# fxcawley/nanoSandbox

Hardware: AMD Instinct MI355X
Metric: tokens/sec (whole node) GPT-2 124M DDP (higher is better)
Workload: dtype bf16

## Files before the change

csrc/kernels/flash_attn.hip:

```cpp
#include "common.h"

#include <type_traits>

#ifndef NSA_FA_F16
#define NSA_FA_F16 0
#endif
#if NSA_FA_F16
#define NSA_FA_SYM(name) name##_h
#else
#define NSA_FA_SYM(name) name
#endif
constexpr bool kFaH = NSA_FA_F16 != 0;

namespace {

__device__ __forceinline__ __bf16 fa_elt(float v) { return f2frag<kFaH>(v); }
__device__ __forceinline__ float fa_f(__bf16 v) { return e2f<kFaH>(__builtin_bit_cast(uint16_t, v)); }

constexpr float kLog2e = 1.4426950408889634f;
#ifndef ATTN_ORDER_DEFAULT
#define ATTN_ORDER_DEFAULT 0
#endif

template <int D>
// ... 4 lines not shown
};

template <int BITS>
__device__ __forceinline__ int bitrev(int k) {
  if constexpr (BITS == 2) return ((k & 1) << 1) | ((k >> 1) & 1);
  else if constexpr (BITS == 3) return ((k & 1) << 2) | (k & 2) | ((k >> 2) & 1);
  else return (int)(__builtin_bitreverse32((uint32_t)k) >> 28);
}

template <int D>
__device__ __forceinline__ int swz(int row, int chunk) {
  using G = Geo<D>;
  const int key = bitrev<G::BITS>((row / G::RPB) & (G::CPR - 1));
  return row * (D * 2) + ((chunk ^ key) << 4);
}

__device__ __forceinline__ uint4 lds_b128(const char* base, int off) {
  return *reinterpret_cast<const uint4*>(base + off);
}

__device__ __forceinline__ s16x4 lds_tr(const char* base, int off) {
  return __builtin_amdgcn_ds_read_tr16_b64_v4i16((__attribute__((address_space(3))) s16x4*)(base + off));
}

__device__ __forceinline__ bf16x8 cat_tr(s16x4 a, s16x4 b) {
  typedef short s16x8 __attribute__((ext_vector_type(8)));
  s16x8 v = __builtin_shufflevector(a, b, 0, 1, 2, 3, 4, 5, 6, 7);
  return __builtin_bit_cast(bf16x8, v);
}

__device__ __forceinline__ bf16x8 as_frag(uint4 u) { return __builtin_bit_cast(bf16x8, u); }

__device__ __forceinline__ f32x16 mfma(bf16x8 a, bf16x8 b, f32x16 c) { return mfma32e<kFaH>(a, b, c); }

__device__ __forceinline__ void attn_order(int n_tiles, int BH, int order, int& bh, int& t) {
  const int v = blockIdx.x;
  if (order == 0) {
    t = v / BH;
    bh = v % BH;
    return;
  }
  if (order == 2) {
    bh = v / n_tiles;
    t = v % n_tiles;
    return;
  }
  const int total = n_tiles * BH;
  const int xcd = v % 8, q = total / 8, r = total % 8;
  const int u = (xcd < r ? xcd * (q + 1) : r * (q + 1) + (xcd - r) * q) + v / 8;
  bh = u / n_tiles;
  t = u % n_tiles;
}

enum { FWD_AUTO = 0, FWD_V1 = 1, FWD_V5 = 5 };
enum { BWD_V1 = 1, BWD_V2 = 2, BWD_V3 = 3 };
struct FlashConfig {
  int fwd, bwd, order;
};
}
NSA_API void* nsa_flash_config_ptr();
namespace {
#if NSA_FA_F16
FlashConfig& flash_config() { return *static_cast<FlashConfig*>(nsa_flash_config_ptr()); }
#else
FlashConfig& flash_config() {
  static FlashConfig c = [] {
    FlashConfig d{FWD_AUTO, BWD_V3, ATTN_ORDER_DEFAULT};
    if (const char* e = getenv("NSA_FLASH_FWD"))
      d.fwd = (e[0] == 'v' && (e[1] == '1' || e[1] == '5')) ? e[1] - '0' : FWD_AUTO;
    if (const char* e = getenv("NSA_FLASH_BWD"))
      d.bwd = (e[0] == 'v' && e[1] >= '1' && e[1] <= '3') ? e[1] - '0' : BWD_V3;
    if (const char* e = getenv("NSA_ATTN_ORDER")) d.order = (e[0] >= '0' && e[0] <= '2') ? e[0] - '0' : 0;
    return d;
  }();
  return c;
}
#endif
int attn_order_env() { return flash_config().order; }

__device__ __forceinline__ int acc_row(int i, int h) { return (i & 3) + 8 * (i >> 2) + 4 * h; }

__device__ __forceinline__ float fast_exp2(float x) { return __builtin_amdgcn_exp2f(x); }

template <int D>
__device__ __forceinline__ bf16x8 tr_frag(const char* tile, int r0, int r1, int col_base, int lane) {
  const int g = lane >> 4, ig = lane & 15;
  const int q = ig >> 2, p = ig & 3;
  const int col = col_base + 16 * (g & 1) + 4 * p;
  const int chunk = col >> 3, half = (col >> 2) & 1;
  const s16x4 a = lds_tr(tile, swz<D>(r0 + q, chunk) + half * 8);
  const s16x4 b = lds_tr(tile, swz<D>(r1 + q, chunk) + half * 8);
  return cat_tr(a, b);
}

template <int W>
__device__ __forceinline__ bf16x8 tr_frag_w(const char* tile, int r0, int r1, int col_base, int lane) {
  return tr_frag<W>(tile, r0, r1, col_base, lane);
}

#ifndef NSA_FA_M0KEEP
#define NSA_FA_M0KEEP 0
#endif
__device__ __forceinline__ void glds16s(uint32_t voff, const void* sbase, uint32_t lds_dst) {
  if constexpr (NSA_FA_M0KEEP) {
    unsigned keep;
    asm volatile("s_mov_b32 %0, m0\n\ts_mov_b32 m0, %3\n\ts_nop 0\n\tglobal_load_lds_dwordx4 %1, %2\n\ts_mov_b32 m0, %0"
                 : "=&s"(keep)
                 : "v"(voff), "s"(sbase), "s"(lds_dst)
                 : "memory");
  } else {
    asm volatile("s_mov_b32 m0, %2\n\ts_nop 0\n\tglobal_load_lds_dwordx4 %0, %1" ::"v"(voff), "s"(sbase), "s"(lds_dst)
                 : "memory");
  }
}
__device__ __forceinline__ void glds16(const void* gsrc, uint32_t lds_dst) {
  if constexpr (NSA_FA_M0KEEP) {
    unsigned keep;
    asm volatile("s_mov_b32 %0, m0\n\ts_mov_b32 m0, %2\n\ts_nop 0\n\tglobal_load_lds_dwordx4 %1, off\n\ts_mov_b32 m0, %0"
                 : "=&s"(keep)
                 : "v"(gsrc), "s"(lds_dst)
                 : "memory");
  } else {
// ... 521 lines not shown
  asm volatile("s_waitcnt vmcnt(0)" ::: "memory");
  __syncthreads();
  for (int j = 0; j < n_tiles; j += 2) {
    issue(min(j + 2, n_tiles - 1), (j + 2) % 4);
    issue(min(j + 3, n_tiles - 1), (j + 3) % 4);
#pragma unroll
    for (int u = 0; u < 2; ++u) {
      const int jj = j + u;
      if (NSA_PROBE_SKIP_TILE && jj == 1) continue;
      if (jj < n_tiles) {
        const int kv0 = jj * BN;
        const char* kt = smem + (jj % 4) * TILE_BYTES;
        const char* vt = smem + (4 + jj % 4) * TILE_BYTES;
        if (kv0 + BN - 1 <= q0w) {
          if (!(fast && fwd_tile5<false>(kt, vt, qf, o, l_i, kv0, qposA, h, r, lane, scale_log2))) {
            if (fast) fwd5_to_exact(o, m_i, l_i, sl_exact);
            fast = false;
            fwd_tile2<false, false>(kt, vt, qf, o, m_i, l_i, kv0, qposA, h, r, lane, sl_exact, dr);
          }
        } else if (kv0 <= q0w + 63) {
          if (!(fast && fwd_tile5<true>(kt, vt, qf, o, l_i, kv0, qposA, h, r, lane, scale_log2))) {
            if (fast) fwd5_to_exact(o, m_i, l_i, sl_exact);
            fast = false;
            fwd_tile2<true, false>(kt, vt, qf, o, m_i, l_i, kv0, qposA, h, r, lane, sl_exact, dr);
          }
        }
      }
    }
    asm volatile("s_waitcnt vmcnt(0)" ::: "memory");
    __syncthreads();
  }
#pragma unroll
  for (int blk = 0; blk < 2; ++blk) {
    const int qp = qposA + 32 * blk;
    if (qp < T) {
      const float inv_l = 1.0f / l_i[blk];
      bf16_t* orow = out + ((int64_t)b * T + qp) * C + hh * D;
#pragma unroll
      for (int dt = 0; dt < 2; ++dt) {
#pragma unroll
        for (int g = 0; g < 4; ++g) {
          const int d = 32 * dt + 8 * g + 4 * h;
          uint2 u;
          u.x = pk2<kFaH>(o[blk][dt][4 * g + 0] * inv_l, o[blk][dt][4 * g + 1] * inv_l);
          u.y = pk2<kFaH>(o[blk][dt][4 * g + 2] * inv_l, o[blk][dt][4 * g + 3] * inv_l);
          *reinterpret_cast<uint2*>(orow + d) = u;
        }
      }
      if (h == 0) lse_out[(int64_t)bh * T + qp] = (m_i[blk] * sl_exact + __log2f(l_i[blk])) * 0.6931471805599453f;
    }
  }
}

template <int D>
__global__ __launch_bounds__(256) void flash_bwd_pre_kernel(const bf16_t* __restrict__ o,
                                                           const bf16_t* __restrict__ dout,
                                                           float* __restrict__ delta, int B, int T, int H) {
  constexpr int LPR = D / 8;
  const int C = H * D;
  const int64_t gid = (int64_t)blockIdx.x * 256 + threadIdx.x;
  const int64_t row = gid / LPR;
  const int sub = gid % LPR;
  if (row >= (int64_t)B * T * H) return;
  const int hh = row % H;
  const int64_t bt = row / H;
  const int t = bt % T, b = bt / T;
  const int64_t off = bt * C + hh * D + sub * 8;
  float a[8], g[8];
  load8e<kFaH>(o + off, a);
  load8e<kFaH>(dout + off, g);
  float s = 0.0f;
#pragma unroll
  for (int j = 0; j < 8; ++j) s += a[j] * g[j];
#pragma unroll
  for (int k = LPR / 2; k > 0; k >>= 1) s += __shfl_xor(s, k, 64);
  if (sub == 0) delta[((int64_t)b * H + hh) * T + t] = s;
}

template <int D>
struct BwdGeo {
  static constexpr int KB = D == 64 ? 256 : 128;
  static constexpr int NW = KB / 32;
};

template <bool MASK, bool DROP>
__device__ __forceinline__ void bwd_probs(const f32x16& sacc, const f32x16& dpacc, const float* lse2_s,
                                          const float* delta_s, int qrow0, int qbase_pos, int kpos, int h,
                                          float scale_log2, const DropArgs& dr, bf16x8 (&pfr)[2],
                                          bf16x8 (&dsfr)[2]) {
#pragma unroll
  for (int g = 0; g < 4; ++g) {
    const float4 l4 = *reinterpret_cast<const float4*>(lse2_s + qrow0 + 8 * g + 4 * h);
    const float4 d4 = *reinterpret_cast<const float4*>(delta_s + qrow0 + 8 * g + 4 * h);
    const float lv[4] = {l4.x, l4.y, l4.z, l4.w};
    const float dlv[4] = {d4.x, d4.y, d4.z, d4.w};
#pragma unroll
    for (int e = 0; e < 4; ++e) {
      const int i = 4 * g + e;
      const int q = qbase_pos + 8 * g + 4 * h + e;
      float p = fast_exp2(sacc[i] * scale_log2 - lv[e]);
      if constexpr (MASK) {
        if (kpos > q || q >= dr.T) p = 0.0f;
      }
      float dp = dpacc[i];
      float pd = p;
      if constexpr (DROP) {
// ... 391 lines not shown
  for (int kb = 0; kb < NKB; ++kb) {
    sacc[kb] = row_consts(ld, h);
#pragma unroll
    for (int ks = 0; ks < 4; ++ks) sacc[kb] = mfma(qa[ks], kf[kb][ks], sacc[kb]);
  }
#pragma unroll
  for (int kb = 0; kb < NKB; ++kb) {
    pacc[kb] = DROP ? f32x16{} : row_consts(ld + 32, h);
#pragma unroll
    for (int ks = 0; ks < 4; ++ks) pacc[kb] = mfma(da[ks], vf[kb][ks], pacc[kb]);
  }
  bf16x8 pfr[NKB][2], dsfr[NKB][2];
#pragma unroll
  for (int kb = 0; kb < NKB; ++kb) {
    const int key = kw + 32 * kb + r;
    f32x16 nd;
    if constexpr (DROP) nd = row_consts(ld + 32, h);
    float pv[16], dsv[16];
#pragma unroll
    for (int i = 0; i < 16; ++i) {
      float p = fast_exp2(sacc[kb][i] * scale_log2);
      if constexpr (MASK) p = key > q0 + acc_row(i, h) ? 0.0f : p;
      if constexpr (DROP) {
        const int q = q0 + acc_row(i, h);
        const uint64_t id = ((uint64_t)dr.bh * dr.T + (uint64_t)q) * (uint64_t)dr.T + (uint64_t)key;
        const bool keep = nsa_keep(dr.seed, id, dr.thresh);
        pv[i] = keep ? p * dr.scale : 0.0f;
        dsv[i] = p * ((keep ? pacc[kb][i] * dr.scale : 0.0f) + nd[i]);
      } else {
        pv[i] = p;
        dsv[i] = p * pacc[kb][i];
      }
    }
    pack16(pv, pfr[kb]);
    pack16(dsv, dsfr[kb]);
  }
#pragma unroll
  for (int s = 0; s < 2; ++s) {
    const int r0 = 16 * s + 4 * h;
#pragma unroll
    for (int dt = 0; dt < 2; ++dt) {
      const bf16x8 doa = tr_frag<D>(dot, r0, r0 + 8, 32 * dt, lane);
#pragma unroll
      for (int kb = 0; kb < NKB; ++kb) dv[kb][dt] = mfma(doa, pfr[kb][s], dv[kb][dt]);
      const bf16x8 qta = tr_frag<D>(qt, r0, r0 + 8, 32 * dt, lane);
#pragma unroll
      for (int kb = 0; kb < NKB; ++kb) dk[kb][dt] = mfma(qta, dsfr[kb][s], dk[kb][dt]);
    }
  }
}

#ifndef NSA_DKDV_NS
#define NSA_DKDV_NS 4
#endif

template <int NKB, int NW, bool DROP, int G = 1>
__global__ __launch_bounds__(NW * 64, NKB == 2 ? 1 : (NW == 8 ? 1 : 2)) void flash_bwd_dkdv2_kernel(
    const bf16_t* __restrict__ qkv, const bf16_t* __restrict__ dout, const float* __restrict__ nls,
    const float* __restrict__ nd, bf16_t* __restrict__ dqkv, int B, int T, int H, float scale,
    float scale_log2, uint32_t drop_thresh, float drop_scale, uint64_t seed, int order) {
  constexpr int D = 64;
  constexpr int KPW = 32 * NKB;
  constexpr int KWG = KPW * NW;
  constexpr int SLOT = V2Geo<NW>::SLOT;
  constexpr int NS = G > 1 ? 2 * G : NSA_DKDV_NS, LA = NS - 1;
  __shared__ __attribute__((aligned(16))) char smem[NS * SLOT];
  const int C = H * D;
  const int64_t row_stride = 3 * (int64_t)C;
  const int BH = B * H;
  int bh, kbw;
  attn_order((T + KWG - 1) / KWG, BH, order, bh, kbw);
  const int b = bh / H, hh = bh % H;
  const int tid = threadIdx.x, lane = tid & 63;
  const int w = __builtin_amdgcn_readfirstlane(tid >> 6);
  const int h = lane >> 5, r = lane & 31;
  const int k0 = kbw * KWG;
  const int kw = k0 + KPW * w;
  const bf16_t* base = qkv + (int64_t)b * T * row_stride;
  const bf16_t* qbase = base + hh * D;
  const bf16_t* kbase = base + C + hh * D;
  const bf16_t* vbase = base + 2 * C + hh * D;
  const bf16_t* dobase = dout + (int64_t)b * T * C + hh * D;
  const float* nls_bh = nls + (int64_t)bh * T;
  const float* nd_bh = nd + (int64_t)bh * T;
  const DropArgs dr{drop_thresh, drop_scale, nsa_seed(seed), bh, T};
  const uint32_t lds0 =
      __builtin_amdgcn_readfirstlane((uint32_t)(uintptr_t)((__attribute__((address_space(3))) char*)smem));

  const int s_first = k0 / 32;
  const int n_mine = T / 32 - s_first;

  const int piece = NW == 4 ? w : (w & 3);
  const int prow = 8 * piece + (lane >> 3);
  const int pch = (lane & 7) ^ bitrev<3>((prow >> 1) & 7);
  const bf16_t* qsrc = qbase + (int64_t)prow * row_stride + pch * 8;
  const bf16_t* dosrc = dobase + (int64_t)prow * C + pch * 8;
  const float* csrc = (h == 0 ? nls_bh : nd_bh) + r;
  auto issue = [&](int s, int slot) {
    const uint32_t sb = lds0 + (uint32_t)(slot * SLOT);
    if (NW == 4 || w < 4) glds16(qsrc + (int64_t)s * 32 * row_stride, sb + (uint32_t)(8 * piece * 128));
    if (NW == 4 || w >= 4) glds16(dosrc + (int64_t)s * 32 * C, sb + (uint32_t)(V2_QT + 8 * piece * 128));
    glds4(csrc + s * 32, sb + (uint32_t)(2 * V2_QT + w * 256));
  };

  for (int j = 0; j < (G > 1 ? G : LA) && j < n_mine; ++j) issue(s_first + j, j);

  bf16x8 kf[NKB][4], vf[NKB][4];
#pragma unroll
  for (int kb = 0; kb < NKB; ++kb) {
    int kc = kw + 32 * kb + r;
    kc = kc < T ? kc : T - 1;
#pragma unroll
    for (int ks = 0; ks < 4; ++ks) {
      kf[kb][ks] = as_frag(*reinterpret_cast<const uint4*>(kbase + (int64_t)kc * row_stride + 16 * ks + 8 * h));
      vf[kb][ks] = as_frag(*reinterpret_cast<const uint4*>(vbase + (int64_t)kc * row_stride + 16 * ks + 8 * h));
    }
  }
#pragma unroll
  for (int kb = 0; kb < NKB; ++kb)
    asm volatile("" ::"v"(kf[kb][0]), "v"(kf[kb][1]), "v"(kf[kb][2]), "v"(kf[kb][3]), "v"(vf[kb][0]),
                 "v"(vf[kb][1]), "v"(vf[kb][2]), "v"(vf[kb][3]));
  f32x16 dk[NKB][2], dv[NKB][2];
#pragma unroll
  for (int kb = 0; kb < NKB; ++kb)
#pragma unroll
    for (int dt = 0; dt < 2; ++dt) {
      dk[kb][dt] = f32x16{};
      dv[kb][dt] = f32x16{};
    }

  auto open_slice = [&](int j) {
    vm_wait(V2Geo<NW>::PIECES * min(LA - 1, n_mine - 1 - j));
    asm volatile("s_waitcnt lgkmcnt(0)" ::: "memory");
    __builtin_amdgcn_s_barrier();
    if (j + LA < n_mine) issue(s_first + j + LA, (j + LA) % NS);
  };
  auto slice_full = [&](int j) {
    auto f = [&](auto slot) {
      const char* qt = smem + decltype(slot)::value * SLOT;
      dkdv_slice<NKB, false, DROP>(qt, qt + V2_QT, reinterpret_cast<const float*>(qt + 2 * V2_QT) + w * 64, kf,
                                   vf, dk, dv, (s_first + j) * 32, kw, h, r, lane, scale_log2, dr);
    };
    slot_dispatch<0, NS>(j % NS, f);
  };
  auto slice_diag = [&](int j) {
    auto f = [&](auto slot) {
      const char* qt = smem + decltype(slot)::value * SLOT;
      dkdv_slice<NKB, true, DROP>(qt, qt + V2_QT, reinterpret_cast<const float*>(qt + 2 * V2_QT) + w * 64, kf,
                                  vf, dk, dv, (s_first + j) * 32, kw, h, r, lane, scale_log2, dr);
    };
    slot_dispatch<0, NS>(j % NS, f);
  };

  const int j_diag = min(NKB * w, n_mine);
  const int j_full = min(NKB * w + NKB, n_mine);
  if constexpr (G > 1) {
    for (int j = 0; j < n_mine; j += G) {
      asm volatile("s_waitcnt vmcnt(0) lgkmcnt(0)" ::: "memory");
      __builtin_amdgcn_s_barrier();
#pragma unroll
      for (int u = 0; u < G; ++u)
        if (j + G + u < n_mine) issue(s_first + j + G + u, (j + G + u) % NS);
#pragma unroll
      for (int u = 0; u < G; ++u) {
        const int jj = j + u;
        if (jj >= j_full) {
          if (jj < n_mine) slice_full(jj);
        } else if (jj >= j_diag) {
          slice_diag(jj);
        }
      }
    }
  } else {
    int j = 0;
    for (; j < j_diag; ++j) open_slice(j);
    for (; j < j_full; ++j) {
      open_slice(j);
      slice_diag(j);
    }
    for (; j < n_mine; ++j) {
      open_slice(j);
      slice_full(j);
    }
  }

#pragma unroll
  for (int kb = 0; kb < NKB; ++kb) {
    const int kpos = kw + 32 * kb + r;
    if (kpos < T) {
      bf16_t* krow = dqkv + ((int64_t)b * T + kpos) * row_stride + C + hh * D;
      bf16_t* vrow = krow + C;
#pragma unroll
      for (int dt = 0; dt < 2; ++dt) {
#pragma unroll
        for (int g = 0; g < 4; ++g) {
          const int d = 32 * dt + 8 * g + 4 * h;
          uint2 uk, uv;
          uk.x = cvt2(dk[kb][dt][4 * g + 0] * scale, dk[kb][dt][4 * g + 1] * scale);
          uk.y = cvt2(dk[kb][dt][4 * g + 2] * scale, dk[kb][dt][4 * g + 3] * scale);
          uv.x = cvt2(dv[kb][dt][4 * g + 0], dv[kb][dt][4 * g + 1]);
          uv.y = cvt2(dv[kb][dt][4 * g + 2], dv[kb][dt][4 * g + 3]);
          *reinterpret_cast<uint2*>(krow + d) = uk;
          *reinterpret_cast<uint2*>(vrow + d) = uv;
        }
      }
    }
  }
}

constexpr int DQ2_T = 64 * 64 * 2;
#ifndef NSA_DQ2_NS
#define NSA_DQ2_NS 4
#endif
#ifndef NSA_DQ2_OCC
#define NSA_DQ2_OCC 2
#endif

template <bool MASK, bool DROP>
__device__ __forceinline__ void dq2_tile(const char* kt, const char* vt, const bf16x8 (&qf)[4],
                                         const bf16x8 (&gf)[4], const f32x16& ndt, f32x16 (&dq)[2], float lse2,
                                         int kv0, int qpos, int h, int r, int lane, float scale_log2,
                                         const DropArgs& dr) {
  constexpr int D = 64;
  f32x16 st[2], pt[2];
#pragma unroll
// ... 128 lines not shown
    auto f = [&](auto slot) {
      const char* kt = smem + decltype(slot)::value * SLOT;
      dq2_tile<false, DROP>(kt, kt + DQ2_T, qf, gf, ndt, dq, lse2, 64 * j, qpos, h, r, lane, scale_log2, dr);
    };
    slot_dispatch<0, NS>(j % NS, f);
  };
  auto tile_diag = [&](int j) {
    auto f = [&](auto slot) {
      const char* kt = smem + decltype(slot)::value * SLOT;
      dq2_tile<true, DROP>(kt, kt + DQ2_T, qf, gf, ndt, dq, lse2, 64 * j, qpos, h, r, lane, scale_log2, dr);
    };
    slot_dispatch<0, NS>(j % NS, f);
  };

  const int m = min(q0w / 64, n_tiles);
  int j = 0;
  for (; j < m; ++j) {
    open_tile(j);
    tile_full(j);
  }
  if (j < n_tiles) {
    open_tile(j);
    tile_diag(j);
    ++j;
  }
  for (; j < n_tiles; ++j) open_tile(j);

  if (qpos < T) {
    bf16_t* qrow = dqkv + ((int64_t)b * T + qpos) * row_stride + hh * D;
#pragma unroll
    for (int dt = 0; dt < 2; ++dt) {
#pragma unroll
      for (int g = 0; g < 4; ++g) {
        const int d = 32 * dt + 8 * g + 4 * h;
        uint2 u;
        u.x = cvt2(dq[dt][4 * g + 0] * scale, dq[dt][4 * g + 1] * scale);
        u.y = cvt2(dq[dt][4 * g + 2] * scale, dq[dt][4 * g + 3] * scale);
        *reinterpret_cast<uint2*>(qrow + d) = u;
      }
    }
  }
}

template <int D>
hipError_t fwd_launch(const void* qkv, void* out, void* lse, int B, int T, int H, float scale, float p,
                      uint64_t seed, hipStream_t s) {
  const int n_qt = (T + 127) / 128;
  const uint32_t th = p > 0.0f ? nsa_drop_thresh(p) : 0u;
  const float dscale = p > 0.0f ? 1.0f / (1.0f - p) : 1.0f;
  const int order = attn_order_env();
  if constexpr (D == 64) {
    const int n_qt5 = (T + 255) / 256;
    const int sel = flash_config().fwd;
    if (!th && (sel == FWD_V5 || (sel == FWD_AUTO && (int64_t)n_qt5 * B * H >= 4096))) {
      flash_fwd5_kernel<<<n_qt5 * B * H, 256, 0, s>>>((const bf16_t*)qkv, (bf16_t*)out, (float*)lse, B, T, H,
                                                      scale * kLog2e, order);
      return hipGetLastError();
    }
    if (th)
      flash_fwd_kernel<D, true, true><<<n_qt * B * H, 256, 0, s>>>((const bf16_t*)qkv, (bf16_t*)out, (float*)lse, B,
                                                                   T, H, scale * kLog2e, th, dscale, seed, order);
    else
      flash_fwd_kernel<D, false, true><<<n_qt * B * H, 256, 0, s>>>((const bf16_t*)qkv, (bf16_t*)out, (float*)lse,
                                                                    B, T, H, scale * kLog2e, th, dscale, seed, order);
    return hipGetLastError();
  }
  if (th)
    flash_fwd_kernel<D, true><<<n_qt * B * H, 256, 0, s>>>((const bf16_t*)qkv, (bf16_t*)out, (float*)lse, B, T, H,
                                                           scale * kLog2e, th, dscale, seed, order);
  else
    flash_fwd_kernel<D, false><<<n_qt * B * H, 256, 0, s>>>((const bf16_t*)qkv, (bf16_t*)out, (float*)lse, B, T, H,
                                                            scale * kLog2e, th, dscale, seed, order);
  return hipGetLastError();
}

template <int D>
hipError_t bwd_launch(const void* qkv, const void* o, const void* dout, const void* lse, void* delta, void* dqkv,
                      int B, int T, int H, float scale, float p, uint64_t seed, hipStream_t s) {
  const int64_t threads = (int64_t)B * T * H * (D / 8);
  flash_bwd_pre_kernel<D><<<(unsigned)((threads + 255) / 256), 256, 0, s>>>((const bf16_t*)o, (const bf16_t*)dout,
                                                                             (float*)delta, B, T, H);
  hipError_t e = hipGetLastError();
  if (e != hipSuccess) return e;
  const uint32_t th = p > 0.0f ? nsa_drop_thresh(p) : 0u;
  const float dscale = p > 0.0f ? 1.0f / (1.0f - p) : 1.0f;
  const int n_kb = (T + BwdGeo<D>::KB - 1) / BwdGeo<D>::KB;
  const dim3 grid(n_kb * B * H), block(BwdGeo<D>::NW * 64);
#define NSA_BWD_ARGS                                                                                        \
  (const bf16_t*)qkv, (const bf16_t*)dout, (const float*)lse, (const float*)delta, (bf16_t*)dqkv, B, T, H, \
      scale, scale * kLog2e, th, dscale, seed
  if (th) flash_bwd_kernel<D, true><<<grid, block, 0, s>>>(NSA_BWD_ARGS);
  else flash_bwd_kernel<D, false><<<grid, block, 0, s>>>(NSA_BWD_ARGS);
#undef NSA_BWD_ARGS
  e = hipGetLastError();
  if (e != hipSuccess) return e;
  const int n_qt = (T + 127) / 128;
  if (th)
    flash_bwd_dq_kernel<D, true><<<n_qt * B * H, 256, 0, s>>>(
        (const bf16_t*)qkv, (const bf16_t*)dout, (const float*)lse, (const float*)delta, (bf16_t*)dqkv, B, T, H,
        scale, scale * kLog2e, th, dscale, seed, 1.0f);
  else
    flash_bwd_dq_kernel<D, false><<<n_qt * B * H, 256, 0, s>>>(
        (const bf16_t*)qkv, (const bf16_t*)dout, (const float*)lse, (const float*)delta, (bf16_t*)dqkv, B, T, H,
        scale, scale * kLog2e, th, dscale, seed, 1.0f);
  return hipGetLastError();
}

// ... 17 lines not shown
  hipError_t e = hipGetLastError();
  if (e != hipSuccess) return e;
  const int n_kb = (T + 127) / 128;
  if (flash_config().bwd == BWD_V3 && !th)
    flash_bwd_dkdv2_kernel<1, 4, false, 2><<<n_kb * B * H, 256, 0, s>>>((const bf16_t*)qkv, (const bf16_t*)dout,
                                                                          nls, nd, (bf16_t*)dqkv, B, T, H, scale,
                                                                          scale * kLog2e, th, dscale, seed, order);
  else if (th)
    flash_bwd_dkdv2_kernel<1, 4, true><<<n_kb * B * H, 256, 0, s>>>((const bf16_t*)qkv, (const bf16_t*)dout, nls, nd,
                                                                   (bf16_t*)dqkv, B, T, H, scale, scale * kLog2e, th,
                                                                   dscale, seed, order);
  else
    flash_bwd_dkdv2_kernel<1, 4, false><<<n_kb * B * H, 256, 0, s>>>((const bf16_t*)qkv, (const bf16_t*)dout, nls,
                                                                    nd, (bf16_t*)dqkv, B, T, H, scale, scale * kLog2e,
                                                                    th, dscale, seed, order);
  return hipGetLastError();
}

}

NSA_API hipError_t NSA_FA_SYM(nsa_flash_bwd2)(const void* qkv, const void* o, const void* dout, const void* lse, void* ws,
                                  void* dqkv, int B, int T, int H, int D, float scale, float p, uint64_t seed,
                                  hipStream_t s) {
  if (D == 64 && T % 32 == 0 && flash_config().bwd >= BWD_V2)
    return bwd2_launch64(qkv, o, dout, lse, ws, dqkv, B, T, H, scale, p, seed, s);
  switch (D) {
    case 32: return bwd_launch<32>(qkv, o, dout, lse, ws, dqkv, B, T, H, scale, p, seed, s);
    case 64: return bwd_launch<64>(qkv, o, dout, lse, ws, dqkv, B, T, H, scale, p, seed, s);
    case 128: return bwd_launch<128>(qkv, o, dout, lse, ws, dqkv, B, T, H, scale, p, seed, s);
    default: return hipErrorInvalidValue;
  }
}

#define NSA_FA_RNG(NAME) NSA_DEFINE_RNG_ADVANCE(NAME)
NSA_FA_RNG(NSA_FA_SYM(nsa_rng_advance_attn))


NSA_API hipError_t NSA_FA_SYM(nsa_flash_fwd)(const void* qkv, void* out, void* lse, int B, int T, int H, int D, float scale,
                                 float p, uint64_t seed, hipStream_t s) {
  switch (D) {
    case 32: return fwd_launch<32>(qkv, out, lse, B, T, H, scale, p, seed, s);
    case 64: return fwd_launch<64>(qkv, out, lse, B, T, H, scale, p, seed, s);
    case 128: return fwd_launch<128>(qkv, out, lse, B, T, H, scale, p, seed, s);
    default: return hipErrorInvalidValue;
  }
}

#if !NSA_FA_F16
NSA_API void* nsa_flash_config_ptr() { return &flash_config(); }

NSA_API int nsa_flash_set_variant(int fwd, int bwd, int order) {
  FlashConfig& c = flash_config();
  const int prev = c.fwd | (c.bwd << 4) | (c.order << 8);
  if (fwd == FWD_AUTO || fwd == FWD_V1 || fwd == FWD_V5) c.fwd = fwd;
  if (bwd >= BWD_V1 && bwd <= BWD_V3) c.bwd = bwd;
  if (order >= 0 && order <= 2) c.order = order;
  return prev;
}
#endif
```

nanosandbox_amd/build.py:

```python

from __future__ import annotations

import argparse
import glob
import os
import shutil
import subprocess
import sys
from concurrent.futures import ThreadPoolExecutor

ROOT = os.path.dirname(os.path.dirname(os.path.abspath(__file__)))
CSRC = os.path.join(ROOT, "csrc")
LIB_DIR = os.path.join(ROOT, "nanosandbox_amd", "lib")
BUILD_DIR = os.path.join(ROOT, "build", "obj")
ARCH = os.environ.get("NSA_OFFLOAD_ARCH", "gfx950")

KERNEL_LIB = os.path.join(LIB_DIR, "libnsa_kernels.so")
RUNTIME_LIB = os.path.join(LIB_DIR, "libnsa_runtime.so")
BIN_DIR = os.path.join(ROOT, "nanosandbox_amd", "bin")
RCCL_BENCH = os.path.join(BIN_DIR, "rccl_bench")


def _hipcc():
    for c in (os.environ.get("HIPCC"), "/opt/rocm/bin/hipcc", shutil.which("hipcc")):
        if c and os.path.exists(c):
            return c
    raise FileNotFoundError("hipcc not found (ROCm 7.x expected under /opt/rocm)")


def _newer(target, sources):
    if not os.path.exists(target):
        return True
    t = os.path.getmtime(target)
    return any(os.path.getmtime(s) > t for s in sources)


def _run(cmd):
    r = subprocess.run(cmd, capture_output=True, text=True)
    if r.returncode != 0:
        raise RuntimeError(f"build failed: {' '.join(cmd)}\n{r.stdout}\n{r.stderr}")
    return r


FILE_FLAGS = {"flash_attn.hip": ["-fno-slp-vectorize"], "flash_attn_f16.hip": ["-fno-slp-vectorize"]}


def build_kernels(force=False, jobs=8, verbose=True, defines=(), lib_path=KERNEL_LIB, obj_dir=BUILD_DIR,
                  file_flags=None):
    srcs = sorted(glob.glob(os.path.join(CSRC, "kernels", "*.hip")))
    headers = glob.glob(os.path.join(CSRC, "kernels", "*.h"))
    if not force and not _newer(lib_path, srcs + headers + [os.path.abspath(__file__)]):
        return lib_path
    os.makedirs(obj_dir, exist_ok=True)
    os.makedirs(os.path.dirname(lib_path), exist_ok=True)
    hipcc = _hipcc()
    flags = [f"--offload-arch={ARCH}", "-O3", "-std=c++17", "-fPIC", "-fvisibility=hidden",
             "-munsafe-fp-atomics", "-I", os.path.join(CSRC, "kernels"), *[f"-D{d}" for d in defines]]

    def deps(src):
        out = []
        for line in open(src):
            if line.startswith('#include "') and line.rstrip().endswith('.hip"'):
                out.append(os.path.join(os.path.dirname(src), line.split('"')[1]))
        return out

    ff = FILE_FLAGS if file_flags is None else file_flags

    def compile_one(src):
        obj = os.path.join(obj_dir, os.path.basename(src) + ".o")
        if force or _newer(obj, [src] + headers + deps(src) + [os.path.abspath(__file__)]):
            _run([hipcc, *flags, *ff.get(os.path.basename(src), []), "-c", src, "-o", obj])
            if verbose:
                print(f"  [hipcc {ARCH}] {os.path.relpath(src, ROOT)}")
        return obj

    with ThreadPoolExecutor(max_workers=max(1, jobs)) as ex:
        objs = list(ex.map(compile_one, srcs))
    tmp = lib_path + ".tmp"
    _run([hipcc, f"--offload-arch={ARCH}", "-shared", "-fPIC", *objs, "-o", tmp])
    os.replace(tmp, lib_path)
    if verbose:
        print(f"built {os.path.relpath(lib_path, ROOT)}")
    return lib_path


def build_variant(name, defines, force=False, jobs=8, verbose=True, file_flags=None):
    vdir = os.path.join(ROOT, "build", "variants", name)
    return build_kernels(force=force, jobs=jobs, verbose=verbose, defines=defines,
                         lib_path=os.path.join(vdir, "libnsa_kernels.so"), obj_dir=os.path.join(vdir, "obj"),
                         file_flags=file_flags)


def build_runtime(force=False, verbose=True):
    srcs = sorted(glob.glob(os.path.join(CSRC, "runtime", "*.cpp")))
    if not srcs:
        return None
    if not force and not _newer(RUNTIME_LIB, srcs):
        return RUNTIME_LIB
    os.makedirs(LIB_DIR, exist_ok=True)
    cxx = os.environ.get("CXX", "g++")
    tmp = RUNTIME_LIB + ".tmp"
    _run([cxx, "-O3", "-std=c++17", "-fPIC", "-shared", "-pthread", *srcs, "-o", tmp])
    os.replace(tmp, RUNTIME_LIB)
    if verbose:
        print(f"built {os.path.relpath(RUNTIME_LIB, ROOT)}")
    return RUNTIME_LIB


def build_tools(force=False, verbose=True):
    src = os.path.join(CSRC, "comm", "rccl_bench.cpp")
    if not os.path.exists(src):
        return None
    if not force and not _newer(RCCL_BENCH, [src]):
        return RCCL_BENCH
    os.makedirs(BIN_DIR, exist_ok=True)
    rocm = os.environ.get("ROCM_PATH", "/opt/rocm")
    tmp = RCCL_BENCH + ".tmp"
    _run([_hipcc(), "-O2", "-std=c++17", "-I", os.path.join(rocm, "include"), src, "-L", os.path.join(rocm, "lib"),
          "-lrccl", f"-Wl,-rpath,{os.path.join(rocm, 'lib')}", "-o", tmp])
    os.replace(tmp, RCCL_BENCH)
    if verbose:
        print(f"built {os.path.relpath(RCCL_BENCH, ROOT)}")
    return RCCL_BENCH


def build_all(force=False, jobs=8, verbose=True):
    build_runtime(force=force, verbose=verbose)
    build_tools(force=force, verbose=verbose)
    return build_kernels(force=force, jobs=jobs, verbose=verbose)


def main(argv=None):
    ap = argparse.ArgumentParser()
    ap.add_argument("--force", action="store_true")
    ap.add_argument("--jobs", type=int, default=min(8, os.cpu_count() or 1))
    ap.add_argument("--variant", nargs="+", metavar=("NAME", "DEFINE"),
                    help="build an A/B probe variant: NAME followed by preprocessor defines")
    ap.add_argument("--no-file-flags", action="store_true",
                    help="with --variant: compile every source with the common flags only (no FILE_FLAGS)")
    a = ap.parse_args(argv)
    if a.variant:
        print(build_variant(a.variant[0], a.variant[1:], force=a.force, jobs=a.jobs,
                            file_flags={} if a.no_file_flags else None))
        return 0
    build_all(force=a.force, jobs=a.jobs)


if __name__ == "__main__":
    sys.exit(main())
```

nanosandbox_amd/ops/functional.py:

```python

from __future__ import annotations

import contextlib
import math
import os
from typing import NamedTuple

import torch
import torch.nn.functional as F

from . import _lib
from . import gemm as _gemm
from . import gemm_dispatch as _gd

BF16 = torch.bfloat16
F16 = torch.float16
F32 = torch.float32
KDT = (BF16, F16)


def _sym(name, dtype):
    return name + "_h" if dtype == F16 else name


# ... 557 lines not shown

def mlp(x, w_fc, b_fc, w_proj, b_proj, recompute=False):
    if x.is_cuda and x.dtype in KDT:
        return MLPFn.apply(x, w_fc, b_fc, w_proj, b_proj, recompute)
    return linear(gelu(linear(x, w_fc, b_fc)), w_proj, b_proj)



_INV_SQRT2 = 1.0 / math.sqrt(2.0)
_INV_SQRT2PI = 1.0 / math.sqrt(2.0 * math.pi)


class GeluFn(torch.autograd.Function):
    @staticmethod
    def forward(ctx, x):
        ctx.save_for_backward(x)
        if _kern(x):
            x = x.contiguous()
            y = torch.empty_like(x)
            _lib.call(_sym("nsa_gelu_fwd", x.dtype), _lib.ptr(x), _lib.ptr(y), x.numel(), _lib.stream())
            return y
        return F.gelu(x.float()).to(x.dtype)

    @staticmethod
    def backward(ctx, dy):
        (x,) = ctx.saved_tensors
        if _kern(dy):
            dy = dy.contiguous()
            dx = torch.empty_like(x)
            _lib.call(_sym("nsa_gelu_bwd", dy.dtype), _lib.ptr(dy), _lib.ptr(x), _lib.ptr(dx), x.numel(), _lib.stream())
            return dx
        xf = x.float()
        cdf = 0.5 * (1.0 + torch.erf(xf * _INV_SQRT2))
        pdf = torch.exp(-0.5 * xf * xf) * _INV_SQRT2PI
        return (dy.float() * (cdf + xf * pdf)).to(dy.dtype)


def gelu(x):
    return GeluFn.apply(x)



def _attn_reference(q, k, v, p, seed):
    T, D = q.shape[-2], q.shape[-1]
    att = (q @ k.transpose(-2, -1)) * (1.0 / math.sqrt(D))
    mask = torch.ones(T, T, dtype=torch.bool, device=q.device).tril()
    att = att.masked_fill(~mask, float("-inf"))
    att = torch.softmax(att, dim=-1)
    if p > 0:
        att = att * _cpu_keep_mask(att.shape, p, seed, att.device) / (1.0 - p)
    return att @ v


_FLASH_FWD = {"auto": 0, "v1": 1, "v5": 5}
_FLASH_BWD = {"v1": 1, "v2": 2, "v3": 3}


@contextlib.contextmanager
def flash_variant(fwd: str | None = None, bwd: str | None = None, order: int | None = None):
    prev = _lib.call_ret("nsa_flash_set_variant", _FLASH_FWD[fwd] if fwd else -1, _FLASH_BWD[bwd] if bwd else -1,
                         -1 if order is None else int(order))
    try:
        yield
    finally:
        _lib.call_ret("nsa_flash_set_variant", prev & 0xF, (prev >> 4) & 0xF, (prev >> 8) & 0xF)


class AttentionFn(torch.autograd.Function):
    @staticmethod
    def forward(ctx, qkv, n_head, p):
        B, T, C3 = qkv.shape
        C = C3 // 3
        H = n_head
        D = C // H
        seed = new_seed() if p > 0 else 0
        ctx.meta = (B, T, H, D, p, seed)
        scale = 1.0 / math.sqrt(D)
        ctx.kern = _kern(qkv)
        if ctx.kern:
            assert D in (32, 64, 128), "flash kernel supports head_dim 32/64/128"
            qkv = qkv.contiguous()
            y = torch.empty(B, T, C, device=qkv.device, dtype=qkv.dtype)
            lse = torch.empty(B, H, T, device=qkv.device, dtype=F32)
            _lib.call(_sym("nsa_flash_fwd", qkv.dtype), _lib.ptr(qkv), _lib.ptr(y), _lib.ptr(lse), B, T, H, D,
                      scale, p, seed, _lib.stream())
            ctx.save_for_backward(qkv, y, lse)
            return y
        q, k, v = qkv.float().view(B, T, 3, H, D).permute(2, 0, 3, 1, 4)
        y = _attn_reference(q, k, v, p, seed).transpose(1, 2).reshape(B, T, C)
        ctx.save_for_backward(qkv)
        return y.to(qkv.dtype)

    @staticmethod
    def backward(ctx, dy):
        B, T, H, D, p, seed = ctx.meta
        C = H * D
        if ctx.kern:
            qkv, y, lse = ctx.saved_tensors
            dy = dy.contiguous()
            dqkv = torch.empty_like(qkv)
            ws = torch.empty(2, B, H, T, device=dy.device, dtype=F32)
            dy = dy.to(qkv.dtype)
            _lib.call(_sym("nsa_flash_bwd2", qkv.dtype), _lib.ptr(qkv), _lib.ptr(y), _lib.ptr(dy), _lib.ptr(lse),
                      _lib.ptr(ws), _lib.ptr(dqkv), B, T, H, D, 1.0 / math.sqrt(D), p, seed, _lib.stream())
            return dqkv, None, None
        (qkv,) = ctx.saved_tensors
        with torch.enable_grad():
# ... 530 lines not shown
```

Baseline: 1.239 million.

## Add fwd8 flash attention kernel with paired causal query blocks as auto default

Adds a new forward flash-attention kernel (v8) where each wave handles two 32-row query blocks paired from opposite ends of a 256-row tile (w and 7-w), balancing causal work across waves. It shares K fragment loads across both blocks and uses compile-time block masks to skip dead and masked sub-tiles. A fast path without running max falls back to an exact online softmax on overflow. Auto dispatch now selects v8 instead of v5, and the change also adds probe instrumentation and build tooling that are off by default.

```diff
diff --git a/csrc/kernels/flash_attn.hip b/csrc/kernels/flash_attn.hip
--- a/csrc/kernels/flash_attn.hip
+++ b/csrc/kernels/flash_attn.hip
@@ -80,7 +80,7 @@
   t = u % n_tiles;
 }
 
-enum { FWD_AUTO = 0, FWD_V1 = 1, FWD_V5 = 5 };
+enum { FWD_AUTO = 0, FWD_V1 = 1, FWD_V5 = 5, FWD_V8 = 8 };
 enum { BWD_V1 = 1, BWD_V2 = 2, BWD_V3 = 3 };
 struct FlashConfig {
   int fwd, bwd, order;
@@ -95,7 +95,7 @@
   static FlashConfig c = [] {
     FlashConfig d{FWD_AUTO, BWD_V3, ATTN_ORDER_DEFAULT};
     if (const char* e = getenv("NSA_FLASH_FWD"))
-      d.fwd = (e[0] == 'v' && (e[1] == '1' || e[1] == '5')) ? e[1] - '0' : FWD_AUTO;
+      d.fwd = (e[0] == 'v' && (e[1] == '1' || e[1] == '5' || e[1] == '8')) ? e[1] - '0' : FWD_AUTO;
     if (const char* e = getenv("NSA_FLASH_BWD"))
       d.bwd = (e[0] == 'v' && e[1] >= '1' && e[1] <= '3') ? e[1] - '0' : BWD_V3;
     if (const char* e = getenv("NSA_ATTN_ORDER")) d.order = (e[0] >= '0' && e[0] <= '2') ? e[0] - '0' : 0;
@@ -723,6 +723,334 @@
   }
 }
 
+enum { BM_VIS = 0, BM_D0 = 1, BM_D1 = 2, BM_OFF = 3 };
+constexpr bool bm_live(int m, int sb) { return m == BM_VIS || m == BM_D1 || (m == BM_D0 && sb == 0); }
+constexpr bool bm_mask(int m, int sb) { return (m == BM_D0 && sb == 0) || (m == BM_D1 && sb == 1); }
+
+struct Fwd8Addr {
+  uint32_t k[4], v[2][2];
+};
+__device__ __forceinline__ Fwd8Addr fwd8_addr(int lane) {
+  Fwd8Addr ad;
+  const int h = lane >> 5, r = lane & 31;
+#pragma unroll
+  for (int ks = 0; ks < 4; ++ks) ad.k[ks] = (uint32_t)swz<64>(r, 2 * ks + h);
+  const int g = lane >> 4, ig = lane & 15;
+  const int q = ig >> 2, p = ig & 3;
+#pragma unroll
+  for (int dt = 0; dt < 2; ++dt) {
+    const int col = 32 * dt + 16 * (g & 1) + 4 * p;
+#pragma unroll
+    for (int x = 0; x < 2; ++x) ad.v[x][dt] = (uint32_t)(swz<64>(4 * h + q + 8 * x, col >> 3) + ((col >> 2) & 1) * 8);
+  }
+  return ad;
+}
+
+template <bool LA, bool LB>
+__device__ __forceinline__ void fwd8_scores(const char* kt, int sb, const bf16x8 (&qf)[2][4], f32x16& sa, f32x16& sb_,
+                                            const Fwd8Addr& ad) {
+  if constexpr (LA || LB) {
+    if constexpr (LA) sa = f32x16{};
+    if constexpr (LB) sb_ = f32x16{};
+#pragma unroll
+    for (int ks = 0; ks < 4; ++ks) {
+      const bf16x8 kf = as_frag(lds_b128(kt, ad.k[ks] + 32 * 128 * sb));
+      if constexpr (LA) sa = mfma(kf, qf[0][ks], sa);
+      if constexpr (LB) sb_ = mfma(kf, qf[1][ks], sb_);
+    }
+  }
+}
+
+template <bool LA, bool LB>
+__device__ __forceinline__ void fwd8_pv(const char* vt, int sb, const bf16x8 (&pa)[2], const bf16x8 (&pb)[2],
+                                        f32x16 (&o)[2][2], const Fwd8Addr& ad) {
+  if constexpr (LA || LB) {
+#pragma unroll
+    for (int s = 0; s < 2; ++s) {
+      const int rows = (32 * sb + 16 * s) * 128;
+#pragma unroll
+      for (int dt = 0; dt < 2; ++dt) {
+        const bf16x8 vf = cat_tr(lds_tr(vt, ad.v[0][dt] + rows), lds_tr(vt, ad.v[1][dt] + rows));
+        if constexpr (LA) o[0][dt] = mfma(vf, pa[s], o[0][dt]);
+        if constexpr (LB) o[1][dt] = mfma(vf, pb[s], o[1][dt]);
+      }
+    }
+  }
+}
+
+template <bool LIVE, bool MASK>
+__device__ __forceinline__ void fwd8_fast_p(f32x16& st, bf16x8 (&pf)[2], float& acc, int h, int r, float scale_log2) {
+  if constexpr (LIVE) {
+    if constexpr (!NSA_FWD5_QSCALE) {
+#pragma unroll
+      for (int i = 0; i < 16; ++i) st[i] *= scale_log2;
+    }
+#pragma unroll
+    for (int i = 0; i < 16; ++i) {
+      float s = st[i];
+      if constexpr (MASK) {
+        if (acc_row(i, h) > r) s = -INFINITY;
+      }
+      const float p = fast_exp2(s);
+      acc += p;
+      pf[i >> 3][i & 7] = fa_elt(p);
+    }
+  }
+}
+
+template <int MA, int MB>
+__device__ __forceinline__ bool fwd_tile8(const char* kt, const char* vt, const bf16x8 (&qf)[2][4], f32x16 (&o)[2][2],
+                                          float (&l_i)[2], const Fwd8Addr& ad, int h, int r, float scale_log2) {
+  f32x16 st[2][2];
+  fwd8_scores<bm_live(MA, 0), bm_live(MB, 0)>(kt, 0, qf, st[0][0], st[1][0], ad);
+  fwd8_scores<bm_live(MA, 1), bm_live(MB, 1)>(kt, 1, qf, st[0][1], st[1][1], ad);
+  bf16x8 pf[2][2][2];
+  float rs[2] = {0.0f, 0.0f};
+  if constexpr (MA != BM_OFF) {
+    float a0 = 0.0f, a1 = 0.0f;
+    fwd8_fast_p<bm_live(MA, 0), bm_mask(MA, 0)>(st[0][0], pf[0][0], a0, h, r, scale_log2);
+    fwd8_fast_p<bm_live(MA, 1), bm_mask(MA, 1)>(st[0][1], pf[0][1], a1, h, r, scale_log2);
+    rs[0] = half_swap_sum(a0 + a1);
+  }
+  if constexpr (MB != BM_OFF) {
+    float a0 = 0.0f, a1 = 0.0f;
+    fwd8_fast_p<bm_live(MB, 0), bm_mask(MB, 0)>(st[1][0], pf[1][0], a0, h, r, scale_log2);
+    fwd8_fast_p<bm_live(MB, 1), bm_mask(MB, 1)>(st[1][1], pf[1][1], a1, h, r, scale_log2);
+    rs[1] = half_swap_sum(a0 + a1);
+  }
+  const float lA = l_i[0] + rs[0], lB = l_i[1] + rs[1];
+  const float hi = kFaH ? 0x1p15f : 0x1p64f, lo = kFaH ? 0x1p-8f : 0x1p-60f;
+  const bool ok = (MA == BM_OFF || (rs[0] <= hi && lA >= lo)) && (MB == BM_OFF || (rs[1] <= hi && lB >= lo));
+  if (__builtin_amdgcn_ballot_w64(!ok)) return false;
+  if constexpr (MA != BM_OFF) l_i[0] = lA;
+  if constexpr (MB != BM_OFF) l_i[1] = lB;
+  fwd8_pv<bm_live(MA, 0), bm_live(MB, 0)>(vt, 0, pf[0][0], pf[1][0], o, ad);
+  fwd8_pv<bm_live(MA, 1), bm_live(MB, 1)>(vt, 1, pf[0][1], pf[1][1], o, ad);
+  return true;
+}
+
+template <int M>
+__device__ __forceinline__ void fwd8_exact_p(f32x16 (&st)[2], bf16x8 (&pf)[2][2], f32x16 (&o)[2], float& m_i,
+                                             float& l_i, int h, int r, float scale_log2) {
+  if constexpr (M != BM_OFF) {
+    float mt = -INFINITY;
+    if constexpr (bm_live(M, 0)) {
+#pragma unroll
+      for (int i = 0; i < 16; ++i) {
+        if constexpr (bm_mask(M, 0)) {
+          if (acc_row(i, h) > r) st[0][i] = -INFINITY;
+        }
+        mt = fmaxf(mt, st[0][i]);
+      }
+    }
+    if constexpr (bm_live(M, 1)) {
+#pragma unroll
+      for (int i = 0; i < 16; ++i) {
+        if constexpr (bm_mask(M, 1)) {
+          if (acc_row(i, h) > r) st[1][i] = -INFINITY;
+        }
+        mt = fmaxf(mt, st[1][i]);
+      }
+    }
+    mt = half_swap_max(mt);
+    const bool grow = (mt - m_i) * scale_log2 > kDeferLog2;
+    if (__builtin_amdgcn_ballot_w64(grow)) {
+      const float m_new = grow ? mt : m_i;
+      const float alpha = fast_exp2((m_i - m_new) * scale_log2);
+      l_i *= alpha;
+      m_i = m_new;
+      o[0] *= alpha;
+      o[1] *= alpha;
+    }
+    const float mc = m_i * scale_log2;
+    float rs = 0.0f;
+    if constexpr (bm_live(M, 0)) {
+#pragma unroll
+      for (int i = 0; i < 16; ++i) {
+        const float p = fast_exp2(st[0][i] * scale_log2 - mc);
+        rs += p;
+        pf[0][i >> 3][i & 7] = fa_elt(p);
+      }
+    }
+    if constexpr (bm_live(M, 1)) {
+#pragma unroll
+      for (int i = 0; i < 16; ++i) {
+        const float p = fast_exp2(st[1][i] * scale_log2 - mc);
+        rs += p;
+        pf[1][i >> 3][i & 7] = fa_elt(p);
+      }
+    }
+    l_i += half_swap_sum(rs);
+  }
+}
+
+template <int MA, int MB>
+__device__ __forceinline__ void fwd_tile8x(const char* kt, const char* vt, const bf16x8 (&qf)[2][4],
+                                           f32x16 (&o)[2][2], float (&m_i)[2], float (&l_i)[2],
+                                           const Fwd8Addr& ad, int h, int r, float scale_log2) {
+  f32x16 st[2][2];
+  fwd8_scores<bm_live(MA, 0), bm_live(MB, 0)>(kt, 0, qf, st[0][0], st[1][0], ad);
+  fwd8_scores<bm_live(MA, 1), bm_live(MB, 1)>(kt, 1, qf, st[0][1], st[1][1], ad);
+  bf16x8 pf[2][2][2];
+  fwd8_exact_p<MA>(st[0], pf[0], o[0], m_i[0], l_i[0], h, r, scale_log2);
+  fwd8_exact_p<MB>(st[1], pf[1], o[1], m_i[1], l_i[1], h, r, scale_log2);
+  fwd8_pv<bm_live(MA, 0), bm_live(MB, 0)>(vt, 0, pf[0][0], pf[1][0], o, ad);
+  fwd8_pv<bm_live(MA, 1), bm_live(MB, 1)>(vt, 1, pf[0][1], pf[1][1], o, ad);
+}
+
+__global__ __launch_bounds__(256, 2) void flash_fwd8_kernel(const bf16_t* __restrict__ qkv, bf16_t* __restrict__ out,
+                                                            float* __restrict__ lse_out, int B, int T, int H,
+                                                            float scale_log2, int order) {
+  constexpr int D = 64;
+  constexpr int BN = 64;
+  constexpr int NS = 4;
+  constexpr int TILE_BYTES = BN * D * 2;
+  __shared__ __attribute__((aligned(16))) char smem[2 * NS * TILE_BYTES];
+
+  const int C = H * D;
+  const int64_t row_stride = 3 * (int64_t)C;
+  const int BH = B * H;
+  const int n_qt = (T + 255) / 256;
+  int bh, qt;
+  attn_order(n_qt, BH, order, bh, qt);
+  qt = n_qt - 1 - qt;
+  const int b = bh / H, hh = bh % H;
+  const int tid = threadIdx.x, lane = tid & 63;
+  const int w = tid >> 6;
+  const int h = lane >> 5, r = lane & 31;
+  const int q0 = qt * 256;
+  const int qpos[2] = {q0 + 32 * w + r, q0 + 32 * (7 - w) + r};
+  const int tA = 4 * qt + (w >> 1), tB = 4 * qt + ((7 - w) >> 1);
+  const bf16_t* base = qkv + (int64_t)b * T * row_stride;
+  const bf16_t* qbase = base + hh * D;
+  const bf16_t* kbase = base + C + hh * D;
+
+  bf16x8 qf[2][4];
+#pragma unroll
+  for (int blk = 0; blk < 2; ++blk) {
+    const int qc = qpos[blk] < T ? qpos[blk] : T - 1;
+#pragma unroll
+    for (int ks = 0; ks < 4; ++ks) {
+      const bf16x8 raw = as_frag(*reinterpret_cast<const uint4*>(qbase + (int64_t)qc * row_stride + 16 * ks + 8 * h));
+#pragma unroll
+      for (int e = 0; e < 8; ++e) qf[blk][ks][e] = NSA_FWD5_QSCALE ? fa_elt(fa_f(raw[e]) * scale_log2) : raw[e];
+    }
+  }
+  f32x16 o[2][2];
+  float m_i[2], l_i[2];
+#pragma unroll
+  for (int blk = 0; blk < 2; ++blk) {
+    o[blk][0] = f32x16{};
+    o[blk][1] = f32x16{};
+    m_i[blk] = 0.0f;
+    l_i[blk] = 0.0f;
+  }
+
+  const int kv_end = min(T, q0 + 256);
+  const int n_tiles = (kv_end + BN - 1) / BN;
+  const uint32_t lds0 =
+      __builtin_amdgcn_readfirstlane((uint32_t)(uintptr_t)((__attribute__((address_space(3))) char*)smem));
+  const int prow = 16 * w + (lane >> 3);
+  const int pch0 = (lane & 7) ^ bitrev<3>((prow >> 1) & 7);
+  const int pch1 = (lane & 7) ^ bitrev<3>(((prow + 8) >> 1) & 7);
+  const uint32_t koff0 = (uint32_t)((prow * (int)row_stride + pch0 * 8) * 2);
+  const uint32_t koff8 = (uint32_t)(((prow + 8) * (int)row_stride + pch1 * 8) * 2);
+  auto issue = [&](int jt, int buf) {
+    const bf16_t* kt_base = kbase + (int64_t)jt * BN * row_stride;
+    uint32_t o0 = koff0, o8 = koff8;
+    if (jt * BN + BN > T) {
+      const int r0 = min(jt * BN + prow, T - 1) - jt * BN, r8 = min(jt * BN + prow + 8, T - 1) - jt * BN;
+      o0 = (uint32_t)((r0 * (int)row_stride + pch0 * 8) * 2);
+      o8 = (uint32_t)((r8 * (int)row_stride + pch1 * 8) * 2);
+    }
+    const uint32_t kb = lds0 + (uint32_t)(buf * TILE_BYTES + 16 * w * 128);
+    const uint32_t vb = kb + NS * TILE_BYTES;
+    glds16s(o0, kt_base, __builtin_amdgcn_readfirstlane(kb));
+    glds16s(o8, kt_base, __builtin_amdgcn_readfirstlane(kb + 1024));
+    glds16s(o0, kt_base + C, __builtin_amdgcn_readfirstlane(vb));
+    glds16s(o8, kt_base + C, __builtin_amdgcn_readfirstlane(vb + 1024));
+  };
+  asm volatile("" ::"v"(qf[0][0]), "v"(qf[0][1]), "v"(qf[0][2]), "v"(qf[0][3]), "v"(qf[1][0]), "v"(qf[1][1]),
+               "v"(qf[1][2]), "v"(qf[1][3]));
+  const float sl_exact = NSA_FWD5_QSCALE ? 1.0f : scale_log2;
+  issue(0, 0);
+  issue(min(1, n_tiles - 1), 1);
+  asm volatile("s_waitcnt vmcnt(0)" ::: "memory");
+  __syncthreads();
+  const Fwd8Addr ad = fwd8_addr(lane);
+  using VIS = std::integral_constant<int, BM_VIS>;
+  using D0 = std::integral_constant<int, BM_D0>;
+  using D1 = std::integral_constant<int, BM_D1>;
+  using OFF = std::integral_constant<int, BM_OFF>;
+  auto dispatch = [&](int jj, auto&& f) -> bool {
+    if (NSA_PROBE_SKIP_TILE && jj == 1) return true;
+    if (jj >= n_tiles || jj > tB) return true;
+    if (jj < tA) return f(jj, VIS{}, VIS{});
+    if (jj == tA) return (w & 1) ? f(jj, D1{}, VIS{}) : f(jj, D0{}, VIS{});
+    if (jj < tB) return f(jj, OFF{}, VIS{});
+    return (w & 1) ? f(jj, OFF{}, D0{}) : f(jj, OFF{}, D1{});
+  };
+  auto fast_tile = [&](int jj, auto ma, auto mb) -> bool {
+    return fwd_tile8<decltype(ma)::value, decltype(mb)::value>(smem + (jj % 4) * TILE_BYTES,
+                                                               smem + (4 + jj % 4) * TILE_BYTES, qf, o, l_i, ad, h,
+                                                               r, scale_log2);
+  };
+  auto exact_tile = [&](int jj, auto ma, auto mb) -> bool {
+    fwd_tile8x<decltype(ma)::value, decltype(mb)::value>(smem + (jj % 4) * TILE_BYTES,
+                                                         smem + (4 + jj % 4) * TILE_BYTES, qf, o, m_i, l_i, ad,
+                                                         h, r, sl_exact);
+    return true;
+  };
+  int j = 0, jx = n_tiles;
+  for (; j < n_tiles; j += 2) {
+    issue(min(j + 2, n_tiles - 1), (j + 2) % 4);
+    issue(min(j + 3, n_tiles - 1), (j + 3) % 4);
+    if (!__builtin_amdgcn_readfirstlane((int)dispatch(j, fast_tile))) {
+      jx = j;
+      break;
+    }
+    if (!__builtin_amdgcn_readfirstlane((int)dispatch(j + 1, fast_tile))) {
+      jx = j + 1;
+      break;
+    }
+    asm volatile("s_waitcnt vmcnt(0)" ::: "memory");
+    __syncthreads();
+  }
+  if (jx < n_tiles) {
+    fwd5_to_exact(o, m_i, l_i, sl_exact);
+    for (;;) {
+      if (j >= jx) dispatch(j, exact_tile);
+      dispatch(j + 1, exact_tile);
+      asm volatile("s_waitcnt vmcnt(0)" ::: "memory");
+      __syncthreads();
+      j += 2;
+      if (j >= n_tiles) break;
+      issue(min(j + 2, n_tiles - 1), (j + 2) % 4);
+      issue(min(j + 3, n_tiles - 1), (j + 3) % 4);
+    }
+  }
+#pragma unroll
+  for (int blk = 0; blk < 2; ++blk) {
+    const int qp = qpos[blk];
+    if (qp < T) {
+      const float inv_l = 1.0f / l_i[blk];
+      bf16_t* orow = out + ((int64_t)b * T + qp) * C + hh * D;
+#pragma unroll
+      for (int dt = 0; dt < 2; ++dt) {
+#pragma unroll
+        for (int g = 0; g < 4; ++g) {
+          const int d = 32 * dt + 8 * g + 4 * h;
+          uint2 u;
+          u.x = pk2<kFaH>(o[blk][dt][4 * g + 0] * inv_l, o[blk][dt][4 * g + 1] * inv_l);
+          u.y = pk2<kFaH>(o[blk][dt][4 * g + 2] * inv_l, o[blk][dt][4 * g + 3] * inv_l);
+          *reinterpret_cast<uint2*>(orow + d) = u;
+        }
+      }
+      if (h == 0) lse_out[(int64_t)bh * T + qp] = (m_i[blk] * sl_exact + __log2f(l_i[blk])) * 0.6931471805599453f;
+    }
+  }
+}
+
 template <int D>
 __global__ __launch_bounds__(256) void flash_bwd_pre_kernel(const bf16_t* __restrict__ o,
                                                            const bf16_t* __restrict__ dout,
@@ -1220,6 +1548,9 @@
 
 #ifndef NSA_DKDV_NS
 #define NSA_DKDV_NS 4
+#endif
+#ifndef NSA_PROBE_DKDV_IDLE
+#define NSA_PROBE_DKDV_IDLE 0
 #endif
 
 template <int NKB, int NW, bool DROP, int G = 1>
@@ -1323,9 +1654,21 @@
   const int j_diag = min(NKB * w, n_mine);
   const int j_full = min(NKB * w + NKB, n_mine);
   if constexpr (G > 1) {
+#if NSA_PROBE_DKDV_IDLE
+    const uint64_t t_start = __builtin_amdgcn_s_memtime();
+    uint64_t t_early = 0, t_rest = 0;
+#endif
     for (int j = 0; j < n_mine; j += G) {
       asm volatile("s_waitcnt vmcnt(0) lgkmcnt(0)" ::: "memory");
+#if NSA_PROBE_DKDV_IDLE
+      const uint64_t t_b = __builtin_amdgcn_s_memtime();
       __builtin_amdgcn_s_barrier();
+      const uint64_t t_w = __builtin_amdgcn_s_memtime() - t_b;
+      if (j > 0 && j - G < j_full) t_early += t_w;
+      else t_rest += t_w;
+#else
+      __builtin_amdgcn_s_barrier();
+#endif
 #pragma unroll
       for (int u = 0; u < G; ++u)
         if (j + G + u < n_mine) issue(s_first + j + G + u, (j + G + u) % NS);
@@ -1339,6 +1682,15 @@
         }
       }
     }
+#if NSA_PROBE_DKDV_IDLE
+    if (lane == 0 && kw < T) {
+      uint64_t* st = reinterpret_cast<uint64_t*>(dqkv + ((int64_t)b * T + kw) * row_stride + hh * D);
+      st[0] = __builtin_amdgcn_s_memtime() - t_start;
+      st[1] = t_early;
+      st[2] = t_rest;
+      st[3] = 0;
+    }
+#endif
   } else {
     int j = 0;
     for (; j < j_diag; ++j) open_slice(j);
@@ -1573,7 +1925,12 @@
   if constexpr (D == 64) {
     const int n_qt5 = (T + 255) / 256;
     const int sel = flash_config().fwd;
-    if (!th && (sel == FWD_V5 || (sel == FWD_AUTO && (int64_t)n_qt5 * B * H >= 4096))) {
+    if (!th && (sel == FWD_V8 || (sel == FWD_AUTO && (int64_t)n_qt5 * B * H >= 4096))) {
+      flash_fwd8_kernel<<<n_qt5 * B * H, 256, 0, s>>>((const bf16_t*)qkv, (bf16_t*)out, (float*)lse, B, T, H,
+                                                      scale * kLog2e, order);
+      return hipGetLastError();
+    }
+    if (!th && sel == FWD_V5) {
       flash_fwd5_kernel<<<n_qt5 * B * H, 256, 0, s>>>((const bf16_t*)qkv, (bf16_t*)out, (float*)lse, B, T, H,
                                                       scale * kLog2e, order);
       return hipGetLastError();
@@ -1697,7 +2054,7 @@
 NSA_API int nsa_flash_set_variant(int fwd, int bwd, int order) {
   FlashConfig& c = flash_config();
   const int prev = c.fwd | (c.bwd << 4) | (c.order << 8);
-  if (fwd == FWD_AUTO || fwd == FWD_V1 || fwd == FWD_V5) c.fwd = fwd;
+  if (fwd == FWD_AUTO || fwd == FWD_V1 || fwd == FWD_V5 || fwd == FWD_V8) c.fwd = fwd;
   if (bwd >= BWD_V1 && bwd <= BWD_V3) c.bwd = bwd;
   if (order >= 0 && order <= 2) c.order = order;
   return prev;
diff --git a/nanosandbox_amd/build.py b/nanosandbox_amd/build.py
--- a/nanosandbox_amd/build.py
+++ b/nanosandbox_amd/build.py
@@ -46,8 +46,10 @@
 
 
 def build_kernels(force=False, jobs=8, verbose=True, defines=(), lib_path=KERNEL_LIB, obj_dir=BUILD_DIR,
-                  file_flags=None):
+                  file_flags=None, only=None):
     srcs = sorted(glob.glob(os.path.join(CSRC, "kernels", "*.hip")))
+    if only is not None:
+        srcs = [s for s in srcs if os.path.basename(s) in only]
     headers = glob.glob(os.path.join(CSRC, "kernels", "*.h"))
     if not force and not _newer(lib_path, srcs + headers + [os.path.abspath(__file__)]):
         return lib_path
@@ -84,11 +86,19 @@
     return lib_path
 
 
-def build_variant(name, defines, force=False, jobs=8, verbose=True, file_flags=None):
+def build_variant(name, defines, force=False, jobs=8, verbose=True, file_flags=None, only=None):
     vdir = os.path.join(ROOT, "build", "variants", name)
     return build_kernels(force=force, jobs=jobs, verbose=verbose, defines=defines,
                          lib_path=os.path.join(vdir, "libnsa_kernels.so"), obj_dir=os.path.join(vdir, "obj"),
-                         file_flags=file_flags)
+                         file_flags=file_flags, only=only)
+
+
+ATTN_SKIP_TILE = ("attn_skip_tile", ["NSA_PROBE_SKIP_TILE=1"], ("flash_attn.hip",))
+
+
+def build_probes(force=False, jobs=8, verbose=True):
+    name, defines, only = ATTN_SKIP_TILE
+    return build_variant(name, defines, force=force, jobs=jobs, verbose=verbose, only=only)
 
 
 def build_runtime(force=False, verbose=True):
@@ -127,6 +137,7 @@
 def build_all(force=False, jobs=8, verbose=True):
     build_runtime(force=force, verbose=verbose)
     build_tools(force=force, verbose=verbose)
+    build_probes(force=force, jobs=jobs, verbose=verbose)
     return build_kernels(force=force, jobs=jobs, verbose=verbose)
 
 
diff --git a/nanosandbox_amd/ops/functional.py b/nanosandbox_amd/ops/functional.py
--- a/nanosandbox_amd/ops/functional.py
+++ b/nanosandbox_amd/ops/functional.py
@@ -633,7 +633,7 @@
     return att @ v
 
 
-_FLASH_FWD = {"auto": 0, "v1": 1, "v5": 5}
+_FLASH_FWD = {"auto": 0, "v1": 1, "v5": 5, "v8": 8}
 _FLASH_BWD = {"v1": 1, "v2": 2, "v3": 3}
 
 
```

Measured after the change: 1.241 million, median of 6. No clear change (+0.1%).
